# Project-Splinter/MonoPort

Hardware: AMD Instinct MI355X
Metric: reconstructions/sec (512^2 in, 256^3 grid) (higher is better)
Workload: dtype f32

## Files before the change

monoport_amd/csrc/api.hip:

```cpp
#include <cstdarg>
#include <cmath>
#include <cstring>

#include "mp_internal.h"
#include "encoder_kernels.h"
#include "octree_common.h"

namespace mp {

static thread_local std::string g_last_error;

int fail(mp_ctx *ctx, int code, const char *fmt, ...) {
  (void)ctx;
  char buf[512];
  va_list ap;
  va_start(ap, fmt);
  vsnprintf(buf, sizeof(buf), fmt, ap);
  va_end(ap);
  g_last_error = buf;
  return code;
}

int ensure_scratch(mp_ctx *ctx, hipStream_t st, size_t bytes, void **out) {
  mp_ctx::Arena &a = ctx->arenas[(void *)st];
// ... 1428 lines not shown
  return keep_largest_checked(ctx, "mp_volume_keep_largest", 1, &volume, r, level, connectivity, fill, &out, &stats,
                              nullptr, stream);
}

int mp_volume_keep_largest_batch(mp_ctx *ctx, int n_frames, const float *const *volume, int r, float level,
                                 int connectivity, float fill, float *const *out, int32_t *const *stats,
                                 const int32_t *const *gate, mp_stream stream) {
  return keep_largest_checked(ctx, "mp_volume_keep_largest_batch", n_frames, volume, r, level, connectivity, fill, out,
                              stats, gate, stream);
}

int mp_group_norm(mp_ctx *ctx, const float *x, int n, int c, int64_t hw, int groups,
                  const float *gamma, const float *beta, float eps, int relu, float *y,
                  mp_stream stream) {
  if (!ctx) return MP_ERR_ARG;
  std::lock_guard<std::mutex> lk(ctx->mu);
  if (!x || !y || !gamma || !beta || n <= 0 || n > 4096 || c <= 0 || hw <= 0 || groups <= 0 ||
      groups > 4096)
    return fail(ctx, MP_ERR_ARG, "mp_group_norm: bad argument");
  if (c % groups || hw % 4 || !aligned16(x) || !aligned16(y))
    return fail(ctx, MP_ERR_UNSUPPORTED, "mp_group_norm: needs C %% groups == 0, HW %% 4 == 0, 16-byte aligned x/y");
  DeviceGuard g(ctx->device);
  void *scratch = nullptr;
  int rc = ensure_scratch(ctx, (hipStream_t)stream, gn_scratch_bytes(n * groups), &scratch);
  if (rc != MP_OK) return rc;
  return launch_group_norm(ctx, scratch, x, n, c, hw, groups, gamma, beta, eps, relu, y,
                           (hipStream_t)stream);
}

int mp_upsample_bicubic2x(mp_ctx *ctx, const float *x, int c, int h, int w, const float *add,
                          float *y, mp_stream stream) {
  if (!ctx) return MP_ERR_ARG;
  std::lock_guard<std::mutex> lk(ctx->mu);
  if (!x || !y || c <= 0 || h < 2 || w < 2)
    return fail(ctx, MP_ERR_ARG, "mp_upsample_bicubic2x: bad argument");
  DeviceGuard g(ctx->device);
  return launch_upsample_bicubic2x(ctx, x, c, h, w, add, y, (hipStream_t)stream);
}

int mp_concat3_add(mp_ctx *ctx, const float *a, int ca, const float *b, int cb, const float *c,
                   int cc, const float *shortcut, int n, int64_t hw, float *y, mp_stream stream) {
  if (!ctx) return MP_ERR_ARG;
  std::lock_guard<std::mutex> lk(ctx->mu);
  if (!a || !b || !c || !shortcut || !y || ca <= 0 || cb <= 0 || cc <= 0 || n <= 0 || hw <= 0)
    return fail(ctx, MP_ERR_ARG, "mp_concat3_add: bad argument");
  if (hw % 4 || !aligned16(a) || !aligned16(b) || !aligned16(c) || !aligned16(shortcut) || !aligned16(y))
    return fail(ctx, MP_ERR_UNSUPPORTED, "mp_concat3_add: needs HW %% 4 == 0 and 16-byte aligned buffers");
  DeviceGuard g(ctx->device);
  return launch_concat3_add(ctx, a, ca, b, cb, c, cc, shortcut, n, hw, y, (hipStream_t)stream);
}

int mp_conv3x3_pack(mp_ctx *ctx, const float *w, int cout, int cin, float *packed, mp_stream stream) {
  if (!ctx) return MP_ERR_ARG;
  std::lock_guard<std::mutex> lk(ctx->mu);
  if (!w || !packed || cout <= 0 || cin <= 0) return fail(ctx, MP_ERR_ARG, "mp_conv3x3_pack: bad argument");
  if (cin % 16 || cout % 32)
    return fail(ctx, MP_ERR_UNSUPPORTED, "mp_conv3x3_pack: needs Cin %% 16 == 0 and Cout %% 32 == 0");
  DeviceGuard g(ctx->device);
  return launch_conv3x3_pack(ctx, w, cout, cin, packed, (hipStream_t)stream);
}

int mp_conv3x3_pack_wino(mp_ctx *ctx, const float *w, int cout, int cin, float *packed_wino, mp_stream stream) {
  if (!ctx) return MP_ERR_ARG;
  std::lock_guard<std::mutex> lk(ctx->mu);
  if (!w || !packed_wino || cout <= 0 || cin <= 0) return fail(ctx, MP_ERR_ARG, "mp_conv3x3_pack_wino: bad argument");
  if (cin % 16 || cout % 32)
    return fail(ctx, MP_ERR_UNSUPPORTED, "mp_conv3x3_pack_wino: needs Cin %% 16 == 0 and Cout %% 32 == 0");
  if (!aligned16(packed_wino)) return fail(ctx, MP_ERR_ARG, "mp_conv3x3_pack_wino: the output must be 16-byte aligned");
  DeviceGuard g(ctx->device);
  return launch_conv3x3_wino_pack(ctx, w, cout, cin, packed_wino, (hipStream_t)stream);
}

int mp_conv3x3_wino_supported(int cin, int cout, int h, int w) { return conv3x3_wino_supported(cin, cout, h, w) ? 1 : 0; }

int mp_conv3x3_pack16(mp_ctx *ctx, const float *w, int cout, int cin, void *packed16, float *wmax,
                      mp_stream stream) {
  if (!ctx) return MP_ERR_ARG;
  std::lock_guard<std::mutex> lk(ctx->mu);
  if (!w || !packed16 || !wmax || cout <= 0 || cin <= 0)
    return fail(ctx, MP_ERR_ARG, "mp_conv3x3_pack16: bad argument");
  if (cin % 16 || cout % 32)
    return fail(ctx, MP_ERR_UNSUPPORTED, "mp_conv3x3_pack16: needs Cin %% 16 == 0 and Cout %% 32 == 0");
  DeviceGuard g(ctx->device);
  return launch_conv3x3_pack16(ctx, w, cout, cin, packed16, wmax, (hipStream_t)stream);
}

int mp_conv3x3_gn16(mp_ctx *ctx, const float *x, int n, int cin, int h, int w, const float *ss, int relu,
                    int reflect, const void *packed16, const float *wmax, int cout, float *y, double *stats,
                    mp_stream stream) {
  if (!ctx) return MP_ERR_ARG;
  std::lock_guard<std::mutex> lk(ctx->mu);
  if (!x || !packed16 || !wmax || !y || n <= 0 || n > 65535 || cin <= 0 || cout <= 0 || h <= 0 || w <= 0)
    return fail(ctx, MP_ERR_ARG, "mp_conv3x3_gn16: bad argument");
  if (!aligned16(packed16)) return fail(ctx, MP_ERR_ARG, "mp_conv3x3_gn16: packed weights must be 16-byte aligned");
  DeviceGuard g(ctx->device);
  return launch_conv3x3_gn(ctx, x, n, cin, h, w, ss, relu, reflect, static_cast<const float *>(packed16),
                           wmax, cout, y, stats, (hipStream_t)stream);
}

int mp_conv1x1_pack(mp_ctx *ctx, const float *w1, int c1, const float *w2, int c2, int cout, int f16,
                    void *packed, float *wmax, mp_stream stream) {
  if (!ctx) return MP_ERR_ARG;
  std::lock_guard<std::mutex> lk(ctx->mu);
  if (!w1 || !packed || c1 <= 0 || c2 < 0 || (c2 > 0 && !w2) || (f16 && !wmax))
    return fail(ctx, MP_ERR_ARG, "mp_conv1x1_pack: bad argument");
  if (c1 % 64 || c2 % 64 || (cout != 128 && cout != 256))
    return fail(ctx, MP_ERR_UNSUPPORTED,
                "mp_conv1x1_pack: input channel counts must be multiples of 64, output channels 128 or 256");
  DeviceGuard g(ctx->device);
  return launch_conv1x1_pack(ctx, w1, c1, w2, c2, cout, f16, packed, wmax, (hipStream_t)stream);
}

int mp_conv1x1(mp_ctx *ctx, const float *x1, const float *ss1, int relu1, const float *x2, int n, int c1,
               int c2, int cout, int64_t hw, const void *packed, int f16, const float *wmax, const float *bias,
               const float *res, float *y, float *y_hwc, double *stats, mp_stream stream) {
  if (!ctx) return MP_ERR_ARG;
  std::lock_guard<std::mutex> lk(ctx->mu);
  if (!x1 || !packed || n <= 0 || hw <= 0 || (!y && !y_hwc) || (f16 && !wmax))
    return fail(ctx, MP_ERR_ARG, "mp_conv1x1: bad argument");
  if (!aligned16(packed) || (y_hwc && !aligned16(y_hwc)))
    return fail(ctx, MP_ERR_ARG, "mp_conv1x1: packed weights / y_hwc must be 16-byte aligned");
  DeviceGuard g(ctx->device);
  return launch_conv1x1_raw(ctx, x1, ss1, relu1, x2, n, c1, c2, cout, hw, packed, f16, wmax, bias, res, y,
                            y_hwc, stats, (hipStream_t)stream);
}

int mp_scale_shift_add(mp_ctx *ctx, const float *t, const float *ss, const float *res, int n, int c,
                       int64_t hw, float *y, mp_stream stream) {
  if (!ctx) return MP_ERR_ARG;
  std::lock_guard<std::mutex> lk(ctx->mu);
  if (!t || !ss || !res || !y || n <= 0 || c <= 0 || hw <= 0)
    return fail(ctx, MP_ERR_ARG, "mp_scale_shift_add: bad argument");
  if (hw % 4 || !aligned16(t) || !aligned16(res) || !aligned16(y))
    return fail(ctx, MP_ERR_UNSUPPORTED, "mp_scale_shift_add: needs HW %% 4 == 0 and 16-byte aligned buffers");
  DeviceGuard g(ctx->device);
  return launch_scale_shift_add(ctx, t, ss, res, (long long)n * c, hw, y, (hipStream_t)stream);
}

int mp_conv3x3_supported(int cin, int cout, int h, int w) { return conv3x3_supported(cin, cout, h, w) ? 1 : 0; }
int mp_conv_stats_supported(int cout) { return conv_stats_supported(cout) ? 1 : 0; }

int mp_gn_stat_slices(void) { return gn_stat_slices(); }

int mp_conv3x3_stat_slices(int cout, int n, int h, int w, int f16) {
  if (cout < 32 || cout % 32 || n < 1 || h < 1 || w < 32) return 0;
  return conv3x3_stat_slices(cout, n, h, w, f16 != 0);
}

void mp_query_tune(int small_tiles) { mp::query_small_set_gate(small_tiles); }

void mp_conv3x3_tune(int nr) {
  conv3x3_set_nr(nr & 0x1fff);
  conv1x1_set_mrw((nr >> 12) & 3);
}

int mp_conv3x3_gn(mp_ctx *ctx, const float *x, int n, int cin, int h, int w, const float *ss, int relu,
                  int reflect, const float *packed, int cout, float *y, double *stats, mp_stream stream) {
  if (!ctx) return MP_ERR_ARG;
  std::lock_guard<std::mutex> lk(ctx->mu);
  if (!x || !packed || !y || n <= 0 || n > 65535 || cin <= 0 || cout <= 0 || h <= 0 || w <= 0)
    return fail(ctx, MP_ERR_ARG, "mp_conv3x3_gn: bad argument");
  if (!aligned16(packed)) return fail(ctx, MP_ERR_ARG, "mp_conv3x3_gn: packed weights must be 16-byte aligned");
  DeviceGuard g(ctx->device);
  return launch_conv3x3_gn(ctx, x, n, cin, h, w, ss, relu, reflect, packed, nullptr, cout, y, stats,
                           (hipStream_t)stream);
}

int mp_gn_stats(mp_ctx *ctx, const float *x, int n, int c, int64_t hw, int groups, double *partial,
                mp_stream stream) {
  if (!ctx) return MP_ERR_ARG;
  std::lock_guard<std::mutex> lk(ctx->mu);
  if (!x || !partial || n <= 0 || c <= 0 || hw <= 0 || groups <= 0)
    return fail(ctx, MP_ERR_ARG, "mp_gn_stats: bad argument");
  if (c % groups || hw % 4 || !aligned16(x))
    return fail(ctx, MP_ERR_UNSUPPORTED, "mp_gn_stats: needs C %% groups == 0, HW %% 4 == 0, 16-byte aligned x");
  DeviceGuard g(ctx->device);
  return launch_gn_stats(ctx, x, n, c, hw, groups, partial, (hipStream_t)stream);
}

int mp_gn_finalize(mp_ctx *ctx, const double *partial, int n, int c, int groups, int slices,
                   int64_t count, const float *gamma, const float *beta, float eps, float *ss,
                   mp_stream stream) {
  if (!ctx) return MP_ERR_ARG;
  std::lock_guard<std::mutex> lk(ctx->mu);
  if (!partial || !gamma || !beta || !ss || n <= 0 || c <= 0 || groups <= 0 || slices <= 0 ||
      count <= 0 || c % groups || c / groups > 64)
    return fail(ctx, MP_ERR_ARG, "mp_gn_finalize: bad argument");
  DeviceGuard g(ctx->device);
  return launch_gn_finalize(ctx, partial, n, c, groups, slices, (double)count, gamma, beta, eps, ss,
                            (hipStream_t)stream);
}

static GnOut to_out(const mp_gn_out *f) {
  GnOut g = gn_out_none();
  if (!f) return g;
  g.acc = reinterpret_cast<long long *>(f->acc);
  g.partial = f->partial;
  return g;
}
static long long out_cap(const mp_gn_out *f) { return f && f->partial ? (long long)f->partial_doubles : -1; }
static GnIn to_in(const mp_gn_in *f) {
  GnIn g = gn_in_none();
  if (!f) return g;
  g.acc = reinterpret_cast<const long long *>(f->acc);
  g.gamma = f->gamma;
  g.beta = f->beta;
  g.eps = f->eps;
  g.ss = f->acc ? nullptr : f->ss;
  return g;
}

int mp_conv3x3_ex(mp_ctx *ctx, const mp_conv3x3_args *q, mp_stream stream) {
  if (!ctx) return MP_ERR_ARG;
  std::lock_guard<std::mutex> lk(ctx->mu);
  if (!q || !q->x || !q->packed || (!q->y && !q->y2) || q->n <= 0 || q->n > 65535 || q->cin <= 0 || q->cout <= 0 ||
      q->h <= 0 || q->w <= 0)
    return fail(ctx, MP_ERR_ARG, "mp_conv3x3_ex: bad argument");
  if (!aligned16(q->packed)) return fail(ctx, MP_ERR_ARG, "mp_conv3x3_ex: packed weights must be 16-byte aligned");
  DeviceGuard g(ctx->device);
  ConvArgs a;
  a.x = q->x;
  a.gn = to_in(&q->gn);
  a.wp = static_cast<const float *>(q->packed);
  a.y = q->y;
  a.y2 = q->y2;
  a.res = q->res;
  a.y2_c = q->y2 ? q->y2_channels : 32;
  a.y2_off = q->y2 ? q->y2_offset : 0;
  a.fin = to_out(&q->fin);
  a.fin2 = to_out(&q->fin2);
  a.n_img = q->n;
  a.cin = q->cin;
  a.cout = q->cout;
  a.h = q->h;
  a.w = q->w;
  a.relu = q->relu;
  a.reflect = q->reflect;
  if (q->packed_wino) {
    if (!aligned16(q->packed_wino)) return fail(ctx, MP_ERR_ARG, "mp_conv3x3_ex: packed_wino must be 16-byte aligned");
    a.wpw = q->packed_wino;
  }
  const long long cap[2] = {out_cap(&q->fin), out_cap(&q->fin2)};
  return launch_conv3x3(ctx, a, q->wmax, cap, (hipStream_t)stream);
}

int mp_conv1x1_ex(mp_ctx *ctx, const mp_conv1x1_args *q, mp_stream stream) {
  if (!ctx) return MP_ERR_ARG;
  std::lock_guard<std::mutex> lk(ctx->mu);
  if (!q || !q->x1 || !q->packed || q->n <= 0 || q->hw <= 0 || (!q->y && !q->y_hwc) || (q->f16 && !q->wmax))
    return fail(ctx, MP_ERR_ARG, "mp_conv1x1_ex: bad argument");
  if (!aligned16(q->packed) || (q->y_hwc && !aligned16(q->y_hwc)))
    return fail(ctx, MP_ERR_ARG, "mp_conv1x1_ex: packed weights / y_hwc must be 16-byte aligned");
  DeviceGuard g(ctx->device);
  Conv1Args a;
  a.x1 = q->x1;
  a.gn1 = to_in(&q->gn1);
  a.x2 = q->x2;
  a.wp = static_cast<const float *>(q->packed);
  a.bias = q->bias;
  a.res = q->res;
  a.y = q->y;
  a.y_hwc = q->y_hwc;
  a.fin = to_out(&q->fin);
  a.n_img = q->n;
  a.c1 = q->c1;
  a.c2 = q->c2;
  a.hw = (int)q->hw;
  a.relu1 = q->relu1;
  a.cout = q->cout;
  return launch_conv1x1(ctx, a, q->f16, q->wmax, out_cap(&q->fin), (hipStream_t)stream);
}

int mp_gn_acc_replicas(void) { return kGnReplicas; }

int mp_conv1x1_stat_slices(int64_t hw) { return hw > 0 ? conv1x1_stat_slices(hw) : 0; }

int mp_convk_supported(int cin, int cout, int ks, int stride, int h, int w) {
  return convk_supported(cin, cout, ks, stride, h, w) ? 1 : 0;
}

int64_t mp_convk_packed_floats(int cin, int cout, int ks) {
  if (cin <= 0 || cout <= 0 || (ks != 3 && ks != 7) || cin % (ks == 7 ? 3 : 16)) return 0;
  return convk_packed_floats(cin, cout, ks);
}

int mp_convk_stat_slices(int ks, int stride, int h, int w) {
  if ((ks != 3 && ks != 7) || stride < 1 || stride > 2 || h <= 0 || w <= 0) return 0;
  return convk_stat_slices(ks, stride, h, w);
}

int mp_convk_pack(mp_ctx *ctx, const float *w, int cout, int cin, int ks, float *packed, mp_stream stream) {
  if (!ctx) return MP_ERR_ARG;
  std::lock_guard<std::mutex> lk(ctx->mu);
  if (!w || !packed || mp_convk_packed_floats(cin, cout, ks) <= 0 || cout % 32)
    return fail(ctx, MP_ERR_ARG, "mp_convk_pack: bad argument");
  DeviceGuard g(ctx->device);
  return launch_convk_pack(ctx, w, cout, cin, ks, packed, (hipStream_t)stream);
}

int mp_convk(mp_ctx *ctx, const mp_convk_args *q, mp_stream stream) {
  if (!ctx) return MP_ERR_ARG;
  std::lock_guard<std::mutex> lk(ctx->mu);
  if (!q || !q->x || !q->packed || !q->y || q->n <= 0 || q->n > 65535 || q->cin <= 0 || q->cout <= 0 ||
      q->h <= 0 || q->w <= 0)
    return fail(ctx, MP_ERR_ARG, "mp_convk: bad argument");
  if (!aligned16(q->packed)) return fail(ctx, MP_ERR_ARG, "mp_convk: packed weights must be 16-byte aligned");
// ... 116 lines not shown
```

monoport_amd/csrc/conv3x3.hip:

```cpp
#include "mp_internal.h"
#include "query_common.h"
#include "gn_tail.h"

namespace mp {

constexpr int kCK = 16;
constexpr int kPixBytes = kCK * 4;
constexpr int kMaxCin = 512;
constexpr int kConvWps = 2;
constexpr int kTileW = 32;
constexpr int halo_pixels(int px) { return (px / kTileW + 2) * (kTileW + 2); }
constexpr int stage_iters(int px) { return (halo_pixels(px) + 63) / 64; }

__global__ void conv3x3_pack_kernel(const float *__restrict__ w, int cout, int cin,
                                    float *__restrict__ wp) {
  const long long total = (long long)cout * cin * 9;
  const int kgt = (cin / kCK) * 18;
  for (long long t = blockIdx.x * (long long)blockDim.x + threadIdx.x; t < total;
       t += (long long)gridDim.x * blockDim.x) {
    const int i = (int)(t & 3), lane = (int)((t >> 2) & 63);
    const long long q = t >> 8;
    const int kg = (int)(q % kgt), rb = (int)(q / kgt);
    const int g = kg & 1, tap = (kg >> 1) % 9, chunk = (kg >> 1) / 9;
    const int co = 32 * rb + (lane & 31);
// ... 1120 lines not shown
  const int swj = j & 15;
  for (int chunk = 0; chunk < n_chunks; ++chunk) {
    const unsigned char *buf = smem + (chunk & 1) * buf_bytes;
    const bool more = chunk + 1 < n_chunks;
    if (more) stage_load(chunk + 1);
#pragma unroll
    for (int s = 0; s < SPC; ++s) {
      const int gs = chunk * SPC + s;
#pragma unroll
      for (int m = 0; m < MRW; ++m)
#pragma unroll
        for (int part = 0; part < FPS; ++part) ring[(s + kAhead) & 3][m][part] = a_load(m, gs + kAhead, part);
      if constexpr (!F16) {
        f32x4 b[2];
#pragma unroll
        for (int n = 0; n < 2; ++n)
          b[n] = *reinterpret_cast<const f32x4 *>(buf + (32 * n + j) * kC1Row + (((2 * s + h) ^ swj) << 4));
        __builtin_amdgcn_sched_barrier(0);
#pragma unroll
        for (int i = 0; i < 4; ++i)
#pragma unroll
          for (int m = 0; m < MRW; ++m)
#pragma unroll
            for (int n = 0; n < 2; ++n)
              acc[m][n] = __builtin_amdgcn_mfma_f32_32x32x2f32(ring[s & 3][m][0][i], b[n][i], acc[m][n], 0, 0, 0);
      } else {
        h8 bh[2], bl[2];
#pragma unroll
        for (int n = 0; n < 2; ++n) {
          const unsigned char *row = buf + (32 * n + j) * kC1Row;
          bh[n] = *reinterpret_cast<const h8 *>(row + (((2 * s + h) ^ swj) << 4));
          bl[n] = *reinterpret_cast<const h8 *>(row + (((8 + 2 * s + h) ^ swj) << 4));
        }
        __builtin_amdgcn_sched_barrier(0);
#pragma unroll
        for (int m = 0; m < MRW; ++m) {
          const h8 ah = __builtin_bit_cast(h8, ring[s & 3][m][0]);
          const h8 al = __builtin_bit_cast(h8, ring[s & 3][m][FPS - 1]);
#pragma unroll
          for (int n = 0; n < 2; ++n)
            acc[m][n] = __builtin_amdgcn_mfma_f32_32x32x16_f16(ah, bh[n], acc[m][n], 0, 0, 0);
#pragma unroll
          for (int n = 0; n < 2; ++n)
            acc[m][n] = __builtin_amdgcn_mfma_f32_32x32x16_f16(ah, bl[n], acc[m][n], 0, 0, 0);
#pragma unroll
          for (int n = 0; n < 2; ++n)
            acc[m][n] = __builtin_amdgcn_mfma_f32_32x32x16_f16(al, bh[n], acc[m][n], 0, 0, 0);
        }
      }
    }
    if (more) stage_store(chunk + 1, smem + ((chunk + 1) & 1) * buf_bytes);
    __syncthreads();
  }

  const float inv_scale = F16 ? 1.0f / conv16_scale(*wmax) : 1.0f;
  constexpr int NCH = 128 * MRW;
  double *cs = reinterpret_cast<double *>(smem);
  const long long img_off = (long long)img * p.cout * p.hw;
  const int img_bytes = p.cout * p.hw * 4;
  const __amdgpu_buffer_rsrc_t rs_res =
      __builtin_amdgcn_make_buffer_rsrc(const_cast<float *>(p.res ? p.res + img_off : p.x1), 0, p.res ? img_bytes : 0, 0x00020000);
  const __amdgpu_buffer_rsrc_t rs_y =
      __builtin_amdgcn_make_buffer_rsrc(p.y ? p.y + img_off : const_cast<float *>(p.x1), 0, p.y ? img_bytes : 0, 0x00020000);
  const int vo = (4 * h * p.hw + px0 + j) * 4;
  auto so_of = [&](int m, int t) { return (32 * (rb0 + m) + (t & 3) + 8 * (t >> 2)) * p.hw * 4; };
#pragma unroll
  for (int m = 0; m < MRW; ++m) {
    float s1[16], s2[16];
#pragma unroll
    for (int t = 0; t < 16; ++t) {
      float b = 0.0f;
      if constexpr (F16) b = p.bias ? p.bias[32 * (rb0 + m) + (t & 3) + 8 * (t >> 2) + 4 * h] : 0.0f;
#pragma unroll
      for (int n = 0; n < 2; ++n) {
        float v = F16 ? acc[m][n][t] * inv_scale + b : acc[m][n][t];
        if (p.res)
          v += __builtin_bit_cast(float, __builtin_amdgcn_raw_buffer_load_b32(rs_res, vo + 128 * n, so_of(m, t), 0));
        acc[m][n][t] = v;
      }
      const float k = half_wave_pivot(acc[m][0][t]);
      const float d0 = acc[m][0][t] - k, d1 = acc[m][1][t] - k;
      s1[t] = d0 + d1;
      s2[t] = fmaf(d1, d1, d0 * d0);
    }
    if (gn_wanted(p.fin)) {
      float k[16];
#pragma unroll
      for (int t = 0; t < 16; ++t) {
        s1[t] = half_wave_sum(s1[t]);
        s2[t] = half_wave_sum(s2[t]);
        k[t] = half_wave_pivot(acc[m][0][t]);
      }
      if (j == kHalfSumLane) {
#pragma unroll
        for (int t = 0; t < 16; ++t) {
          const int lc = 32 * (MRW * wv + m) + (t & 3) + 8 * (t >> 2) + 4 * h;
          gn_unpivot(s1[t], s2[t], k[t], 64.0, cs[2 * lc], cs[2 * lc + 1]);
        }
      }
    }
  }
  if (gn_wanted(p.fin)) {
    __syncthreads();
    if (tid < 64) {
      const int cpg = p.cout / 32, ng = NCH / cpg;
      double a = 0.0, b = 0.0;
      if (tid < ng)
        for (int ch = 0; ch < cpg; ++ch) {
          a += cs[2 * (tid * cpg + ch)];
          b += cs[2 * (tid * cpg + ch) + 1];
        }
      gn_emit(p.fin, img, (NCH * (int)blockIdx.y) / cpg, ng, tile, a, b);
    }
  }
  if (p.y) {
#pragma unroll
    for (int m = 0; m < MRW; ++m)
#pragma unroll
      for (int t = 0; t < 16; ++t) {
#pragma unroll
        for (int n = 0; n < 2; ++n)
        {
          const float v = acc[m][n][t];
          __builtin_amdgcn_raw_buffer_store_b32(__float_as_int(v), rs_y, vo + 128 * n, so_of(m, t), 0);
        }
      }
  }
  if (p.y_hwc) {
    if (gn_wanted(p.fin)) __syncthreads();
    constexpr int kRow = NCH * 4, kSlots = NCH / 4;
    unsigned char *tr = smem;
#pragma unroll
    for (int m = 0; m < MRW; ++m)
#pragma unroll
      for (int n = 0; n < 2; ++n) {
        const int px = 32 * n + j;
#pragma unroll
        for (int q = 0; q < 4; ++q) {
          const int slot = (32 * (MRW * wv + m) + 8 * q + 4 * h) >> 2;
          const f32x4 v = {acc[m][n][4 * q], acc[m][n][4 * q + 1], acc[m][n][4 * q + 2], acc[m][n][4 * q + 3]};
          *reinterpret_cast<f32x4 *>(tr + px * kRow + ((slot ^ (px & (kSlots - 1))) << 4)) = v;
        }
      }
    __syncthreads();
    float *dst = p.y_hwc + ((long long)img * p.hw + px0) * p.cout + NCH * (int)blockIdx.y;
    if (lane < kSlots)
      for (int px = wv; px < kC1Px; px += 4) {
        const f32x4 v = *reinterpret_cast<const f32x4 *>(tr + px * kRow + ((lane ^ (px & (kSlots - 1))) << 4));
        *reinterpret_cast<f32x4 *>(dst + (long long)px * p.cout + 4 * lane) = v;
      }
  }
}

int launch_conv1x1_pack(mp_ctx *ctx, const float *w1, int c1, const float *w2, int c2, int cout, int f16,
                        void *wp, float *wmax, hipStream_t st) {
  const long long total = (long long)cout * (c1 + c2);
  long long blocks = (total + 255) / 256;
  if (blocks > 2048) blocks = 2048;
  if (!f16) {
    hipLaunchKernelGGL(conv1x1_pack_kernel, dim3((unsigned)blocks), dim3(256), 0, st, w1, c1, w2, c2, cout,
                       static_cast<float *>(wp));
  } else {
    MP_HIP(ctx, hipMemsetAsync(wmax, 0, sizeof(float), st));
    int rc = launch_absmax_accumulate(ctx, w1, (long long)cout * c1, reinterpret_cast<unsigned int *>(wmax), st);
    if (rc == MP_OK && c2 > 0)
      rc = launch_absmax_accumulate(ctx, w2, (long long)cout * c2, reinterpret_cast<unsigned int *>(wmax), st);
    if (rc != MP_OK) return rc;
    hipLaunchKernelGGL(conv1x1_pack16_kernel, dim3((unsigned)blocks), dim3(256), 0, st, w1, c1, w2, c2, cout,
                       wmax, static_cast<_Float16 *>(wp));
  }
  MP_HIP(ctx, hipGetLastError());
  return MP_OK;
}

static int g_conv1_mrw = 0;

void conv1x1_set_mrw(int mrw) { g_conv1_mrw = mrw; }

int conv1x1_stat_slices(long long hw) { return (int)(hw / kC1Px); }

int launch_conv1x1(mp_ctx *ctx, Conv1Args a, int f16, const float *wmax, long long partial_cap, hipStream_t st) {
  if (a.c1 <= 0 || a.c1 % kC1K || a.c2 < 0 || a.c2 % kC1K || a.hw % kC1Px || (a.c2 > 0) != (a.x2 != nullptr) ||
      (a.cout != 256 && a.cout != 128))
    return fail(ctx, MP_ERR_UNSUPPORTED,
                "conv1x1: needs C1, C2 multiples of 64, H*W a multiple of 64 and 128 or 256 output channels "
                "(got %d + %d -> %d, %d)", a.c1, a.c2, a.cout, a.hw);
  if (a.c1 > 512)
    return fail(ctx, MP_ERR_UNSUPPORTED, "conv1x1: at most 512 channels in segment 1 (got %d)", a.c1);
  if (a.cout != 256 && (gn_wanted(a.fin) || a.y_hwc))
    return fail(ctx, MP_ERR_UNSUPPORTED, "conv1x1: statistics / channels-last output are built for 256 channels");
  a.wp_floats = a.cout * (a.c1 + a.c2);
  const int tiles = a.hw / kC1Px;
  if (gn_wanted(a.fin)) {
    a.fin.c = a.cout;
    a.fin.S = tiles;
    a.fin.n = a.n_img;
    if (a.fin.partial && partial_cap >= 0 && partial_cap < (long long)a.n_img * 32 * tiles * 2)
      return fail(ctx, MP_ERR_ARG, "conv1x1: statistics buffer holds %lld doubles, the launch writes %lld",
                  partial_cap, (long long)a.n_img * 32 * tiles * 2);
  }
  if (gn_active(a.gn1)) {
    if (a.gn1.acc && (!a.gn1.gamma || !a.gn1.beta))
      return fail(ctx, MP_ERR_ARG, "conv1x1: GroupNorm hand-over without gamma / beta");
    a.gn1.c = a.c1;
    a.gn1.n = a.n_img;
    a.gn1.count = (double)(a.c1 / 32) * a.hw;
  }
  int mrw = 1;
  if (g_conv1_mrw > 0 && a.cout == 256) mrw = g_conv1_mrw;
  const int lds = a.y_hwc ? kC1Px * 512 * mrw : 2 * kC1Px * kC1Row;
  void (*kern)(Conv1Args, const float *) =
      mrw == 2 ? (f16 ? conv1x1_kernel<true, 2> : conv1x1_kernel<false, 2>)
               : (f16 ? conv1x1_kernel<true, 1> : conv1x1_kernel<false, 1>);
  int rc = raise_lds_limit(ctx, reinterpret_cast<const void *>(kern), kC1Px * 1024);
  if (rc != MP_OK) return rc;
  const dim3 grid((unsigned)(tiles * a.n_img), (unsigned)(a.cout / (128 * mrw)));
  hipLaunchKernelGGL(kern, grid, dim3(256), lds, st, a, wmax);
  MP_HIP(ctx, hipGetLastError());
  return MP_OK;
}

int launch_conv1x1_raw(mp_ctx *ctx, const float *x1, const float *ss1, int relu1, const float *x2, int n,
                       int c1, int c2, int cout, long long hw, const void *wp, int f16, const float *wmax,
                       const float *bias, const float *res, float *y, float *y_hwc, double *stats,
                       hipStream_t st) {
  Conv1Args a;
  a.x1 = x1;
  a.gn1 = gn_in_none();
  a.gn1.ss = ss1;
  a.x2 = x2;
  a.wp = static_cast<const float *>(wp);
  a.bias = bias;
  a.res = res;
  a.y = y;
  a.y_hwc = y_hwc;
  a.fin = gn_out_none();
  a.fin.partial = stats;
  a.n_img = n;
  a.c1 = c1;
  a.c2 = c2;
  a.hw = (int)hw;
  a.relu1 = relu1;
  a.cout = cout;
  return launch_conv1x1(ctx, a, f16, wmax, -1, st);
}

}
```

monoport_amd/csrc/encoder_kernels.h:

```cpp
#pragma once
#include "mp_internal.h"

namespace mp {

constexpr int kGnReplicas = 16;

struct GnOut {
  long long *acc;
  double *partial;
  int c;
  int S;
  int n;
};

__host__ __device__ inline GnOut gn_out_none() { return GnOut{nullptr, nullptr, 32, 0, 1}; }
__host__ __device__ inline bool gn_wanted(const GnOut &f) { return f.acc || f.partial; }

struct GnIn {
  const long long *acc;
  const float *gamma, *beta;
  const float *ss;
  float eps;
  int c;
  int n;
  double count;
};

__host__ __device__ inline GnIn gn_in_none() { return GnIn{nullptr, nullptr, nullptr, nullptr, 1e-5f, 32, 1, 1.0}; }
__host__ __device__ inline bool gn_active(const GnIn &g) { return g.acc || g.ss; }

struct ConvArgs {
  const float *x;
  GnIn gn;
  const float *wp;
  float *y;
  float *y2;
  const float *res;
  int y2_c, y2_off;
  GnOut fin;
  GnOut fin2;
  int n_img, cin, cout, h, w;
  int tw, th;
  int relu;
  int reflect;
  int wp_floats;
  const float *wpw = nullptr;
  int wpw_floats = 0;
};

struct Conv1Args {
  const float *x1;
  GnIn gn1;
  const float *x2;
  const float *wp;
  const float *bias;
  const float *res;
  float *y;
  float *y_hwc;
  GnOut fin;
  int n_img, c1, c2, hw, relu1, wp_floats;
  int cout;
};


bool conv3x3_wino_supported(int cin, int cout, int h, int w);
int conv3x3_wino_tiles(int h, int w);
long long conv3x3_wino_workgroups(const ConvArgs &a);
void conv3x3_wino_set_variant(int v);
bool conv3x3_wino_forced();
int launch_conv3x3_wino_pack(mp_ctx *ctx, const float *w, int cout, int cin, float *up, hipStream_t st);
int launch_conv3x3_wino(mp_ctx *ctx, const ConvArgs &a, hipStream_t st);
struct ConvKArgs {
  const float *x;
  GnIn gn;
  const float *wp;
  const float *bias;
  float *y;
  GnOut fin;
  int n_img, cin, cout, h, w, ho, wo;
  int ks, stride, pad, reflect, relu;
  int wp_floats;
};

int launch_conv3x3(mp_ctx *ctx, ConvArgs a, const float *wmax16, const long long partial_cap[2], hipStream_t st);
int launch_conv1x1(mp_ctx *ctx, Conv1Args a, int f16, const float *wmax, long long partial_cap, hipStream_t st);
int conv1x1_stat_slices(long long hw);
void conv1x1_set_mrw(int mrw);
bool convk_supported(int cin, int cout, int ks, int stride, int h, int w);
long long convk_packed_floats(int cin, int cout, int ks);
int convk_stat_slices(int ks, int stride, int h, int w);
int launch_convk_pack(mp_ctx *ctx, const float *w, int cout, int cin, int ks, float *wp, hipStream_t st);
int launch_convk(mp_ctx *ctx, ConvKArgs a, long long partial_cap, hipStream_t st);
int launch_avgpool2_gn(mp_ctx *ctx, const float *x, int n, int c, int h, int w, float *y, GnOut fin,
                       long long partial_cap, hipStream_t st);
bool upsample_gn_banded(int c, int h, int w);
int launch_upsample_add_gn(mp_ctx *ctx, const float *x, int n, int c, int h, int w, const float *add, float *y,
                           GnOut fin, long long partial_cap, hipStream_t st);
int launch_gn_apply_gn(mp_ctx *ctx, const float *x, GnIn gn, int relu, int n, int c, long long hw,
                       const float *res, float *y, GnOut fin, long long partial_cap, hipStream_t st);

}
```

monoport_amd/csrc/gn_tail.h:

```cpp
#pragma once
#include <type_traits>

#include "encoder_kernels.h"

namespace mp {

constexpr int kHalfSumLane = 16;
__device__ __forceinline__ float half_wave_sum(float v) {
  auto dpp = [](float x, auto ctrl_tag) {
    constexpr int ctrl = decltype(ctrl_tag)::value;
    return __builtin_bit_cast(float, __builtin_amdgcn_update_dpp(0, __builtin_bit_cast(int, x), ctrl, 0xF, 0xF, true));
  };
  v += dpp(v, std::integral_constant<int, 0xB1>{});
  v += dpp(v, std::integral_constant<int, 0x4E>{});
  v += dpp(v, std::integral_constant<int, 0x141>{});
  v += dpp(v, std::integral_constant<int, 0x140>{});
  v += __builtin_bit_cast(float, __builtin_amdgcn_update_dpp(0, __builtin_bit_cast(int, v), 0x142, 0xA, 0xF, false));
  return v;
}


__device__ __forceinline__ float half_wave_pivot(float v) {
  int x = __builtin_amdgcn_update_dpp(0, __builtin_bit_cast(int, v), 0x150, 0xF, 0xF, false);
  x = __builtin_amdgcn_update_dpp(x, x, 0x142, 0xA, 0xF, false);
  return __builtin_bit_cast(float, x);
}

__device__ __forceinline__ void gn_unpivot(float s1, float s2, float k, double n, double &a, double &b) {
  const double dk = k, d1 = s1;
  a = d1 + n * dk;
  b = (double)s2 + 2.0 * dk * d1 + n * dk * dk;
}

__device__ __forceinline__ void gn_unpivot_d(double e1, double e2, float k, double n, double &a, double &b) {
  const double dk = k;
  a = e1 + n * dk;
  b = e2 + 2.0 * dk * e1 + n * dk * dk;
}

__device__ __forceinline__ void gn_fixed(double x, long long &hi, unsigned long long &lo) {
  const double xs = x * 65536.0;
  const double fl = floor(xs);
  hi = (long long)fl;
  lo = (unsigned long long)((xs - fl) * 281474976710656.0);
}

__device__ __forceinline__ double gn_unfixed(long long hi, unsigned long long lo) {
  return (double)hi * (1.0 / 65536.0) + (double)lo * (1.0 / 18446744073709551616.0);
}

__device__ __forceinline__ void gn_acc_add(long long *dst_ll, double a, double b) {
  unsigned long long *dst = reinterpret_cast<unsigned long long *>(dst_ll);
  long long hi;
  unsigned long long lo;
  gn_fixed(a, hi, lo);
  (void)__hip_atomic_fetch_add(dst, (unsigned long long)hi, __ATOMIC_RELAXED, __HIP_MEMORY_SCOPE_AGENT);
  (void)__hip_atomic_fetch_add(dst + 1, lo, __ATOMIC_RELAXED, __HIP_MEMORY_SCOPE_AGENT);
  gn_fixed(b, hi, lo);
  (void)__hip_atomic_fetch_add(dst + 2, (unsigned long long)hi, __ATOMIC_RELAXED, __HIP_MEMORY_SCOPE_AGENT);
  (void)__hip_atomic_fetch_add(dst + 3, lo, __ATOMIC_RELAXED, __HIP_MEMORY_SCOPE_AGENT);
}

__device__ __forceinline__ void gn_emit(const GnOut &f, int img, int g0, int ng, int slot, double a, double b) {
  const int tid = threadIdx.x;
  if (tid < ng) {
    if (f.acc)
      gn_acc_add(f.acc + (((long long)(slot % kGnReplicas) * f.n + img) * 32 + g0 + tid) * 4, a, b);
    if (f.partial) {
      double *dst = f.partial + (((long long)img * 32 + g0 + tid) * f.S + slot) * 2;
      dst[0] = a;
      dst[1] = b;
    }
  }
}

__device__ __forceinline__ void gn_mean_rstd(const GnIn &g, const unsigned long long (&w)[4], float &mean,
                                             float &rstd) {
  const double s = gn_unfixed((long long)w[0], w[1]);
  const double q = gn_unfixed((long long)w[2], w[3]);
  const double mean_d = s / g.count;
  const double var_d = fmax(q / g.count - mean_d * mean_d, 0.0);
  mean = (float)mean_d;
  rstd = (float)(1.0 / sqrt(var_d + (double)g.eps));
}

__device__ __forceinline__ void gn_load_stats(const GnIn &g, int img, float *lds_stats ) {
  if (!g.acc) return;
  const int tid = threadIdx.x;
  const int grp = (tid >> 3) & 31, part = tid & 7;
  unsigned long long w[4] = {0, 0, 0, 0};
  for (int r = part; r < kGnReplicas; r += 8) {
    const unsigned long long *a =
        reinterpret_cast<const unsigned long long *>(g.acc) + (((long long)r * g.n + img) * 32 + grp) * 4;
#pragma unroll
    for (int k = 0; k < 4; ++k) w[k] += a[k];
  }
#pragma unroll
  for (int k = 0; k < 4; ++k)
#pragma unroll
    for (int o = 1; o < 8; o <<= 1) w[k] += __shfl_xor(w[k], o);
  if (part == 0 && tid < 256) {
    float mean, rstd;
    gn_mean_rstd(g, w, mean, rstd);
    lds_stats[2 * grp] = mean;
    lds_stats[2 * grp + 1] = rstd;
  }
}

__device__ __forceinline__ void gn_scale_shift(const GnIn &g, int img, int c, const float *lds_stats, float &sc,
                                               float &sh) {
  if (g.acc) {
    const int grp = c / (g.c / 32);
    const float mean = lds_stats[2 * grp], rstd = lds_stats[2 * grp + 1];
    sc = rstd * g.gamma[c];
    sh = g.beta[c] - mean * sc;
  } else if (g.ss) {
    sc = g.ss[2 * ((long long)img * g.c + c)];
    sh = g.ss[2 * ((long long)img * g.c + c) + 1];
  } else {
    sc = 1.0f;
    sh = 0.0f;
  }
}

struct GnAffine {
  float g[2], b[2];
};
__device__ __forceinline__ void gn_affine_load(const GnIn &gn, int channels, GnAffine &a) {
#pragma unroll
  for (int i = 0; i < 2; ++i) {
    const int c = threadIdx.x + 256 * i;
    a.g[i] = a.b[i] = 0.0f;
    if (gn.acc && c < channels) {
      a.g[i] = gn.gamma[c];
      a.b[i] = gn.beta[c];
    }
  }
}
__device__ __forceinline__ void gn_table_fill(const GnIn &gn, int img, int channels, const float *lds_stats,
                                              const GnAffine &a, float *ss ) {
#pragma unroll
  for (int i = 0; i < 2; ++i) {
    const int c = threadIdx.x + 256 * i;
    if (c < channels) {
      float sc, sh;
      if (gn.acc) {
        const int grp = c / (gn.c / 32);
        const float mean = lds_stats[2 * grp], rstd = lds_stats[2 * grp + 1];
        sc = rstd * a.g[i];
        sh = a.b[i] - mean * sc;
      } else {
        gn_scale_shift(gn, img, c, lds_stats, sc, sh);
      }
      ss[2 * c] = sc;
      ss[2 * c + 1] = sh;
    }
  }
}

}
```

Measured before the change: 221.6.

## Add persistent weight-stationary conv1x1 kernel with heuristic routing

Adds a persistent conv1x1 kernel that keeps each wave's weight slice in registers for the whole run. It loops over pixel tiles with double-buffered LDS staging of the GroupNorm-transformed input, overlaps the next tile's global load with the current MFMA work, and defers the GroupNorm statistics emission by two tiles. A heuristic routes selected f32 shapes (mostly layers with GroupNorm applied to the input) to this kernel by default, and a tune knob can force or disable it. The aim is to stop reloading weights for every tile and to hide load latency. In exchange it adds register pressure, a fixed grid sized to the CU count, and another code path that must stay numerically consistent.

Result: no change. 222.8, median of 6 (+0.6%).

```diff
diff --git a/monoport_amd/csrc/api.hip b/monoport_amd/csrc/api.hip
--- a/monoport_amd/csrc/api.hip
+++ b/monoport_amd/csrc/api.hip
@@ -1604,6 +1604,7 @@
 void mp_conv3x3_tune(int nr) {
   conv3x3_set_nr(nr & 0x1fff);
   conv1x1_set_mrw((nr >> 12) & 3);
+  conv1x1_set_route((nr >> 14) & 3, (nr >> 16) & 0xfff);
 }
 
 int mp_conv3x3_gn(mp_ctx *ctx, const float *x, int n, int cin, int h, int w, const float *ss, int relu,
diff --git a/monoport_amd/csrc/conv3x3.hip b/monoport_amd/csrc/conv3x3.hip
--- a/monoport_amd/csrc/conv3x3.hip
+++ b/monoport_amd/csrc/conv3x3.hip
@@ -1296,6 +1296,227 @@
   }
 }
 
+template <int NW, int KC>
+__global__ __launch_bounds__(64 * NW) void conv1x1_ws_kernel(Conv1Args p) {
+  extern __shared__ __attribute__((aligned(16))) unsigned char smem[];
+  constexpr int kRowB = KC * 4;
+  constexpr int kBuf = kC1Px * kRowB;
+  constexpr int CPW = KC / NW;
+  constexpr int NQ = CPW / 4;
+  constexpr int NS = KC / 8;
+  constexpr int NCH = 32 * NW;
+  static_assert(CPW % 4 == 0 && NS % 2 == 0, "conv1x1_ws_kernel: K split");
+  __shared__ float gn_stats[64];
+  __shared__ __attribute__((aligned(16))) float ss1[2 * KC];
+  __shared__ __attribute__((aligned(16))) float bias_s[NCH];
+  __shared__ double cs_s[3][2 * NCH];
+
+  const int tid = threadIdx.x;
+  const int lane = tid & 63;
+  const int wv = __builtin_amdgcn_readfirstlane(tid >> 6);
+  const int tiles = p.hw / kC1Px;
+  const long long total = (long long)tiles * p.n_img;
+  const int t0 = (int)(total * blockIdx.x / gridDim.x), t1 = (int)(total * (blockIdx.x + 1) / gridDim.x);
+  if (t0 >= t1) return;
+
+  f32x4 wr[NS];
+  {
+    const f32x4 *wp4 = reinterpret_cast<const f32x4 *>(p.wp) + (long long)wv * NS * 64 + lane;
+#pragma unroll
+    for (int s = 0; s < NS; ++s) wr[s] = wp4[s * 64];
+  }
+  if (tid < NCH) bias_s[tid] = p.bias ? p.bias[tid] : 0.0f;
+
+  f32x4 stg[NQ];
+  auto stage_load = [&](int img, int px0, int lv) {
+    const __amdgpu_buffer_rsrc_t rs_x = __builtin_amdgcn_make_buffer_rsrc(
+        const_cast<float *>(p.x1 + (long long)img * KC * p.hw), 0, KC * p.hw * 4, 0x00020000);
+#pragma unroll
+    for (int q = 0; q < NQ; ++q)
+#pragma unroll
+      for (int k = 0; k < 4; ++k)
+        stg[q][k] = __builtin_bit_cast(
+            float, __builtin_amdgcn_raw_buffer_load_b32(rs_x, lv * 4, ((CPW * wv + 4 * q + k) * p.hw + px0) * 4, 0));
+  };
+  auto stage_store = [&](unsigned char *buf, int lv) {
+    unsigned char *row = buf + lv * kRowB;
+    const int sw = lv & 15;
+    const bool act = p.relu1 != 0;
+#pragma unroll
+    for (int q = 0; q < NQ; ++q) {
+      const f32x4 ta = *reinterpret_cast<const f32x4 *>(ss1 + 2 * (CPW * wv + 4 * q));
+      const f32x4 tb = *reinterpret_cast<const f32x4 *>(ss1 + 2 * (CPW * wv + 4 * q) + 4);
+      const float sc[4] = {ta[0], ta[2], tb[0], tb[2]}, sh[4] = {ta[1], ta[3], tb[1], tb[3]};
+      f32x4 v;
+#pragma unroll
+      for (int k = 0; k < 4; ++k) {
+        const float t = fmaf(stg[q][k], sc[k], sh[k]);
+        v[k] = act ? fmaxf(t, 0.0f) : t;
+      }
+      *reinterpret_cast<f32x4 *>(row + (((NQ * wv + q) & ~15) << 4) + ((((NQ * wv + q) & 15) ^ sw) << 4)) = v;
+    }
+  };
+  auto emit_stats = [&](int par, int img, int tile, int tv) {
+    if (tv < 32) {
+      constexpr int cpg = NCH / 32;
+      double a = 0.0, b = 0.0;
+      for (int ch = 0; ch < cpg; ++ch) {
+        a += cs_s[par][2 * (tv * cpg + ch)];
+        b += cs_s[par][2 * (tv * cpg + ch) + 1];
+      }
+      if (p.fin.acc)
+        gn_acc_add(p.fin.acc + (((long long)(tile % kGnReplicas) * p.fin.n + img) * 32 + tv) * 4, a, b);
+      if (p.fin.partial) {
+        double *dst = p.fin.partial + (((long long)img * 32 + tv) * p.fin.S + tile) * 2;
+        dst[0] = a;
+        dst[1] = b;
+      }
+    }
+  };
+
+  auto table_build = [&](int img, int tv) {
+    GnAffine affine;
+    gn_affine_load(p.gn1, KC, affine, tv);
+    gn_load_stats(p.gn1, img, gn_stats, tv);
+    __syncthreads();
+    gn_table_fill(p.gn1, img, KC, gn_stats, affine, ss1, tv);
+    __syncthreads();
+  };
+  int img_tab = t0 / tiles;
+  stage_load(img_tab, (t0 % tiles) * kC1Px, lane);
+  table_build(img_tab, tid);
+  stage_store(smem, lane);
+  __syncthreads();
+
+  const bool want_stats = gn_wanted(p.fin);
+  const bool late = !p.y_hwc && wv >= NW / 2;
+  for (int t = t0; t < t1; ++t) {
+    const int par = (t - t0) & 1, slot3 = (t - t0) % 3;
+    const int img = t / tiles, tile = t % tiles;
+    const int px0 = tile * kC1Px;
+    const unsigned char *buf = smem + par * kBuf;
+    const bool more = t + 1 < t1;
+    const int img_n = (t + 1) / tiles;
+    int tv = tid;
+    asm volatile("" : "+v"(tv));
+    const int lv = tv & 63;
+    const int j = lv & 31, h = lv >> 5, swj = lv & 15;
+    if (more) stage_load(img_n, ((t + 1) % tiles) * kC1Px, lv);
+    if (want_stats && t >= t0 + 2) emit_stats((t - 2 - t0) % 3, (t - 2) / tiles, (t - 2) % tiles, tv);
+
+    f32x16 acc[2];
+#pragma unroll
+    for (int q = 0; q < 4; ++q) {
+      const f32x4 b4 = *reinterpret_cast<const f32x4 *>(bias_s + 32 * wv + 8 * q + 4 * h);
+#pragma unroll
+      for (int k = 0; k < 4; ++k) acc[0][4 * q + k] = acc[1][4 * q + k] = b4[k];
+    }
+    int boff[8];
+#pragma unroll
+    for (int q = 0; q < 8; ++q) boff[q] = j * kRowB + (((2 * q + h) ^ swj) << 4);
+    auto b_load = [&](int s, int n) {
+      return *reinterpret_cast<const f32x4 *>(buf + boff[s & 7] + (s >> 3) * 256 + 32 * n * kRowB);
+    };
+    f32x4 b[2][2];
+#pragma unroll
+    for (int n = 0; n < 2; ++n) b[0][n] = b_load(0, n);
+#pragma unroll
+    for (int s = 0; s < NS; ++s) {
+      if (s + 1 < NS) {
+#pragma unroll
+        for (int n = 0; n < 2; ++n)
+          b[(s + 1) & 1][n] = b_load(s + 1, n);
+      }
+      __builtin_amdgcn_sched_barrier(0);
+#pragma unroll
+      for (int i = 0; i < 4; ++i)
+#pragma unroll
+        for (int n = 0; n < 2; ++n)
+          acc[n] = __builtin_amdgcn_mfma_f32_32x32x2f32(wr[s][i], b[s & 1][n][i], acc[n], 0, 0, 0);
+    }
+
+    __builtin_amdgcn_sched_barrier(0);
+    if (more) {
+      if (img_n != img_tab) {
+        table_build(img_n, tv);
+        img_tab = img_n;
+      }
+      stage_store(smem + (par ^ 1) * kBuf, lv);
+    }
+    __builtin_amdgcn_sched_barrier(0);
+    if (late) __syncthreads();
+
+    const long long img_off = (long long)img * NCH * p.hw;
+    const int img_bytes = NCH * p.hw * 4;
+    const __amdgpu_buffer_rsrc_t rs_res =
+        __builtin_amdgcn_make_buffer_rsrc(const_cast<float *>(p.res ? p.res + img_off : p.x1), 0, p.res ? img_bytes : 0, 0x00020000);
+    const __amdgpu_buffer_rsrc_t rs_y =
+        __builtin_amdgcn_make_buffer_rsrc(p.y ? p.y + img_off : const_cast<float *>(p.x1), 0, p.y ? img_bytes : 0, 0x00020000);
+    const int vo = (4 * h * p.hw + px0 + j) * 4;
+    auto so_of = [&](int t16) { return (32 * wv + (t16 & 3) + 8 * (t16 >> 2)) * p.hw * 4; };
+    if (p.res) {
+#pragma unroll
+      for (int t16 = 0; t16 < 16; ++t16)
+#pragma unroll
+        for (int n = 0; n < 2; ++n)
+          acc[n][t16] += __builtin_bit_cast(float, __builtin_amdgcn_raw_buffer_load_b32(rs_res, vo + 128 * n, so_of(t16), 0));
+    }
+    __builtin_amdgcn_sched_barrier(0);
+    if (want_stats) {
+      double *cs = cs_s[slot3];
+#pragma unroll
+      for (int t16 = 0; t16 < 16; ++t16) {
+        const float k = half_wave_pivot(acc[0][t16]);
+        const float d0 = acc[0][t16] - k, d1 = acc[1][t16] - k;
+        const float s1 = half_wave_sum(d0 + d1);
+        const float s2 = half_wave_sum(fmaf(d1, d1, d0 * d0));
+        if (j == kHalfSumLane) {
+          const int lc = 32 * wv + (t16 & 3) + 8 * (t16 >> 2) + 4 * h;
+          gn_unpivot(s1, s2, k, 64.0, cs[2 * lc], cs[2 * lc + 1]);
+        }
+      }
+    }
+    if (p.y) {
+#pragma unroll
+      for (int t16 = 0; t16 < 16; ++t16)
+#pragma unroll
+        for (int n = 0; n < 2; ++n) {
+          const float v = acc[n][t16];
+          __builtin_amdgcn_raw_buffer_store_b32(__float_as_int(v), rs_y, vo + 128 * n, so_of(t16), 0);
+        }
+    }
+    if constexpr (KC == NCH) {
+      if (p.y_hwc) {
+        constexpr int kRow = NCH * 4, kSlots = NCH / 4;
+        __syncthreads();
+        unsigned char *tr = smem + par * kBuf;
+#pragma unroll
+        for (int n = 0; n < 2; ++n) {
+          const int px = 32 * n + j;
+#pragma unroll
+          for (int q = 0; q < 4; ++q) {
+            const int slot = (32 * wv + 8 * q + 4 * h) >> 2;
+            const f32x4 v = {acc[n][4 * q], acc[n][4 * q + 1], acc[n][4 * q + 2], acc[n][4 * q + 3]};
+            *reinterpret_cast<f32x4 *>(tr + px * kRow + ((slot ^ (px & (kSlots - 1))) << 4)) = v;
+          }
+        }
+        __syncthreads();
+        float *dst = p.y_hwc + ((long long)img * p.hw + px0) * NCH;
+        if (lv < kSlots)
+          for (int px = wv; px < kC1Px; px += NW) {
+            const f32x4 v = *reinterpret_cast<const f32x4 *>(tr + px * kRow + ((lv ^ (px & (kSlots - 1))) << 4));
+            *reinterpret_cast<f32x4 *>(dst + (long long)px * NCH + 4 * lv) = v;
+          }
+      }
+    }
+    if (!late) __syncthreads();
+  }
+  if (want_stats) {
+    __syncthreads();
+    for (int t = max(t0, t1 - 2); t < t1; ++t) emit_stats((t - t0) % 3, t / tiles, t % tiles, tid);
+  }
+}
+
 int launch_conv1x1_pack(mp_ctx *ctx, const float *w1, int c1, const float *w2, int c2, int cout, int f16,
                         void *wp, float *wmax, hipStream_t st) {
   const long long total = (long long)cout * (c1 + c2);
@@ -1319,7 +1540,54 @@
 
 static int g_conv1_mrw = 0;
 
+static int g_conv1_route = 0;
+static int g_conv1_ws_cap = 0;
+
 void conv1x1_set_mrw(int mrw) { g_conv1_mrw = mrw; }
+void conv1x1_set_route(int route, int ws_cap) {
+  g_conv1_route = route;
+  g_conv1_ws_cap = ws_cap;
+}
+
+static bool conv1x1_ws_admits(const Conv1Args &a, int f16) {
+  if (f16 || a.c2 != 0 || (a.c1 != 64 && a.c1 != 128 && a.c1 != 256)) return false;
+  if (a.cout == 128 && a.c1 == 256) return false;
+  if (a.y_hwc && a.c1 != 256) return false;
+  return true;
+}
+
+static bool conv1x1_ws_wins(const Conv1Args &a, long long tiles_total, int resident) {
+  if (tiles_total < resident) return false;
+  if (a.c1 == 256 && a.cout == 256 && gn_active(a.gn1) && a.res && !a.y_hwc) return true;
+  if (a.c1 == 64 && a.cout == 128 && gn_active(a.gn1) && !a.res) return true;
+  const bool large = tiles_total >= 32LL * resident;
+  if (a.c1 == 256 && a.cout == 256 && gn_active(a.gn1) && a.y_hwc && !a.res && !gn_wanted(a.fin)) return large;
+  if (a.c1 == 128 && a.cout == 256 && gn_active(a.gn1) && !a.res && !gn_wanted(a.fin) && !a.y_hwc) return large;
+  return false;
+}
+
+template <int NW, int KC>
+static int launch_conv1x1_ws_t(mp_ctx *ctx, const Conv1Args &a, hipStream_t st) {
+  void (*kern)(Conv1Args) = conv1x1_ws_kernel<NW, KC>;
+  const int lds = 2 * kC1Px * KC * 4;
+  int rc = raise_lds_limit(ctx, reinterpret_cast<const void *>(kern), lds);
+  if (rc != MP_OK) return rc;
+  int grid = ctx->n_cu * (NW == 8 ? 1 : 2);
+  if (g_conv1_ws_cap > 0 && grid > g_conv1_ws_cap) grid = g_conv1_ws_cap;
+  hipLaunchKernelGGL(kern, dim3((unsigned)grid), dim3(64 * NW), lds, st, a);
+  MP_HIP(ctx, hipGetLastError());
+  return MP_OK;
+}
+
+static int launch_conv1x1_ws(mp_ctx *ctx, const Conv1Args &a, hipStream_t st) {
+  if (a.cout == 256) {
+    if (a.c1 == 256) return launch_conv1x1_ws_t<8, 256>(ctx, a, st);
+    if (a.c1 == 128) return launch_conv1x1_ws_t<8, 128>(ctx, a, st);
+    return launch_conv1x1_ws_t<8, 64>(ctx, a, st);
+  }
+  if (a.c1 == 128) return launch_conv1x1_ws_t<4, 128>(ctx, a, st);
+  return launch_conv1x1_ws_t<4, 64>(ctx, a, st);
+}
 
 int conv1x1_stat_slices(long long hw) { return (int)(hw / kC1Px); }
 
@@ -1352,6 +1620,15 @@
   }
   int mrw = 1;
   if (g_conv1_mrw > 0 && a.cout == 256) mrw = g_conv1_mrw;
+  const bool ws_ok = conv1x1_ws_admits(a, f16);
+  if (g_conv1_route == 2 && !ws_ok)
+    return fail(ctx, MP_ERR_UNSUPPORTED,
+                "conv1x1: the weight-stationary kernel takes f32, one K segment of 64 / 128 / 256 channels "
+                "(got %d + %d -> %d%s)", a.c1, a.c2, a.cout, f16 ? ", f16x3" : "");
+  if (g_conv1_route == 2 ||
+      (g_conv1_route == 0 && mrw != 2 && ws_ok &&
+       conv1x1_ws_wins(a, (long long)tiles * a.n_img, ctx->n_cu * (a.cout == 256 ? 1 : 2))))
+    return launch_conv1x1_ws(ctx, a, st);
   const int lds = a.y_hwc ? kC1Px * 512 * mrw : 2 * kC1Px * kC1Row;
   void (*kern)(Conv1Args, const float *) =
       mrw == 2 ? (f16 ? conv1x1_kernel<true, 2> : conv1x1_kernel<false, 2>)
diff --git a/monoport_amd/csrc/encoder_kernels.h b/monoport_amd/csrc/encoder_kernels.h
--- a/monoport_amd/csrc/encoder_kernels.h
+++ b/monoport_amd/csrc/encoder_kernels.h
@@ -86,6 +86,7 @@
 int launch_conv1x1(mp_ctx *ctx, Conv1Args a, int f16, const float *wmax, long long partial_cap, hipStream_t st);
 int conv1x1_stat_slices(long long hw);
 void conv1x1_set_mrw(int mrw);
+void conv1x1_set_route(int route, int ws_cap);
 bool convk_supported(int cin, int cout, int ks, int stride, int h, int w);
 long long convk_packed_floats(int cin, int cout, int ks);
 int convk_stat_slices(int ks, int stride, int h, int w);
diff --git a/monoport_amd/csrc/gn_tail.h b/monoport_amd/csrc/gn_tail.h
--- a/monoport_amd/csrc/gn_tail.h
+++ b/monoport_amd/csrc/gn_tail.h
@@ -84,9 +84,8 @@
   rstd = (float)(1.0 / sqrt(var_d + (double)g.eps));
 }
 
-__device__ __forceinline__ void gn_load_stats(const GnIn &g, int img, float *lds_stats ) {
+__device__ __forceinline__ void gn_load_stats(const GnIn &g, int img, float *lds_stats , int tid) {
   if (!g.acc) return;
-  const int tid = threadIdx.x;
   const int grp = (tid >> 3) & 31, part = tid & 7;
   unsigned long long w[4] = {0, 0, 0, 0};
   for (int r = part; r < kGnReplicas; r += 8) {
@@ -105,6 +104,9 @@
     lds_stats[2 * grp] = mean;
     lds_stats[2 * grp + 1] = rstd;
   }
+}
+__device__ __forceinline__ void gn_load_stats(const GnIn &g, int img, float *lds_stats ) {
+  gn_load_stats(g, img, lds_stats, (int)threadIdx.x);
 }
 
 __device__ __forceinline__ void gn_scale_shift(const GnIn &g, int img, int c, const float *lds_stats, float &sc,
@@ -126,10 +128,10 @@
 struct GnAffine {
   float g[2], b[2];
 };
-__device__ __forceinline__ void gn_affine_load(const GnIn &gn, int channels, GnAffine &a) {
+__device__ __forceinline__ void gn_affine_load(const GnIn &gn, int channels, GnAffine &a, int tid) {
 #pragma unroll
   for (int i = 0; i < 2; ++i) {
-    const int c = threadIdx.x + 256 * i;
+    const int c = tid + 256 * i;
     a.g[i] = a.b[i] = 0.0f;
     if (gn.acc && c < channels) {
       a.g[i] = gn.gamma[c];
@@ -137,11 +139,14 @@
     }
   }
 }
+__device__ __forceinline__ void gn_affine_load(const GnIn &gn, int channels, GnAffine &a) {
+  gn_affine_load(gn, channels, a, (int)threadIdx.x);
+}
 __device__ __forceinline__ void gn_table_fill(const GnIn &gn, int img, int channels, const float *lds_stats,
-                                              const GnAffine &a, float *ss ) {
+                                              const GnAffine &a, float *ss , int tid) {
 #pragma unroll
   for (int i = 0; i < 2; ++i) {
-    const int c = threadIdx.x + 256 * i;
+    const int c = tid + 256 * i;
     if (c < channels) {
       float sc, sh;
       if (gn.acc) {
@@ -158,4 +163,9 @@
   }
 }
 
+__device__ __forceinline__ void gn_table_fill(const GnIn &gn, int img, int channels, const float *lds_stats,
+                                              const GnAffine &a, float *ss ) {
+  gn_table_fill(gn, img, channels, lds_stats, a, ss, (int)threadIdx.x);
 }
+
+}
```
